# Ghoul-tn/DSTAGNN_Drought

Measured on AMD Instinct MI355X. Metric: DSTAGNN_block fwd+bwd samples/sec (B,N=170,T=12) @1/2/4/8 GPU; %HBM roofline, higher is better.
Workload: dtype fp32; 1 GPU; PEMS08 inner DSTAGNN_block fwd+bwd (train mode, dropout 0.05); global_batch=32, per_gpu_batch=32, N=170, T=12, F=32, K=3, n_heads=3, d_model=512, d_k=32, parallelism=dp1

## Files before the change

dstagnn_drought_amd/csrc/block.hip:

```cpp
#include <algorithm>
#include <atomic>
#include <vector>
#include <cstring>
#include <mutex>
#include <string>

#include "common.hpp"
#include <chrono>
#include <cstdio>
#include <initializer_list>
#include <map>
#include <utility>
#include "ops.hpp"
#include "streams.hpp"

static thread_local std::string g_last_error;
void set_last_error(const std::string& s) { g_last_error = s; }

namespace {

struct Arena {
  char* base;
  size_t off = 0;
  explicit Arena(void* b) : base((char*)b) {}
  float* take(size_t floats) {
    off = (off + 255) & ~size_t(255);
    float* p = base ? (float*)(base + off) : nullptr;
    off += floats * sizeof(float);
    return p;
  }
};

constexpr size_t kGemmWs = size_t(8) << 20;
constexpr size_t kPart = size_t(2) << 20;

struct Dims {
  int B, N, F, T, h, dk, dv, D, K, C;
  int64_t FT, BFT, BN, NN, HQ, HV, QW, KD, KC, CT, KCT, S;
  int Tg[3], ks[3];
  bool first, sparse, flash;
  bool fsmall;
  bool agg;
  bool dth;
  bool tfused;
  int NP;
  bool tfused_bwd;
  bool gfused;
  bool gbfused;
  int64_t tf_wg;
  int64_t nnz;
  int64_t apa_nnz;
};

Dims mkdims(const dstagnn_block_dims& d) {
  Dims m;
  m.B = d.B; m.N = d.N; m.F = d.F; m.T = d.T; m.h = d.n_heads; m.dk = d.d_k; m.dv = d.d_v;
  m.D = d.d_model; m.K = d.K; m.C = d.C;
  m.FT = (int64_t)m.F * m.T; m.BFT = (int64_t)m.B * m.FT; m.BN = (int64_t)m.B * m.N; m.NN = (int64_t)m.N * m.N;
  m.HQ = (int64_t)m.h * m.dk; m.HV = (int64_t)m.h * m.dv; m.QW = 2 * m.HQ + m.HV; m.KD = (int64_t)m.K * m.dk;
  m.KC = (int64_t)m.K * m.C; m.CT = (int64_t)m.C * m.T; m.KCT = m.KC * m.T; m.S = 3 * (int64_t)m.T - 12;
  for (int g = 0; g < 3; ++g) { m.ks[g] = 3 + 2 * g; m.Tg[g] = m.T - m.ks[g] + 1; }
  m.first = (m.F == 1);
  m.sparse = d.cheb_sparse != 0;
  m.flash = m.sparse && d.cheb_flash != 0;
  m.nnz = m.flash ? d.cheb_nnz : 0;
  m.fsmall = m.flash && flash_small(m.N);
  static const bool agg_env = env_flag("DSTAGNN_CHEB_AGG", true);
  m.agg = agg_env && m.sparse && cheb_agg_ok(m.F, m.C, m.K, m.T);
  m.dth = m.agg && cheb_agg_dtheta_fused(m.B, m.N, m.F, m.C, m.K, m.T, (int64_t)kGemmWs);
  m.apa_nnz = m.fsmall ? std::max(d.cheb_apa_nnz, 0) : 0;
  m.tfused = tat_fused_fwd_ok(m.N, m.T, m.h, m.dk, m.dv);
  m.NP = m.tfused ? tat_fused_np(m.N) : 0;
  m.tfused_bwd = m.tfused && tat_fused_bwd_ok(m.N, m.T, m.h, m.dk, m.dv, m.F, d.res_mode);
  m.tf_wg = m.tfused_bwd ? tat_fused_bwd_wgs(m.BFT) : 0;
  m.gfused = gtu_fused_fwd_ok(m.C, m.T);
  m.gbfused = gtu_fused_bwd_ok(m.C, m.T);
  return m;
}

struct SaveBufs {
  float *Wqkv, *Wqk, *Wp, *thcat, *Wgf[3], *Wgb[3];
  float* Wqkv_p;
  float *WfcT, *WqT;
  float* Wgt[3];
  float *E, *qkv, *att, *ctx, *u_tat, *mu_tat, *rs_tat, *O, *u_s, *mu_s, *rs_s, *Zd, *qk, *P, *W, *xth, *X;
  float *lse, *psupp, *wsupp;
  float *am, *amt, *papa;
  float* conv[3];
  float *G, *tco, *r, *mu_c, *rs_c, *u_et, *mu_et, *rs_et;
};

SaveBufs plan_save(const Dims& m, Arena& a) {
  SaveBufs s;
  s.Wqkv = a.take(m.QW * m.N);
  s.Wqkv_p = m.tfused ? a.take(m.QW * m.NP) : nullptr;
  s.WfcT = m.tfused_bwd ? a.take(m.HV * m.NP) : nullptr;
  s.WqT = m.tfused_bwd ? a.take(m.QW * m.NP) : nullptr;
  for (int g = 0; g < 3; ++g) s.Wgt[g] = m.gfused ? a.take(2 * (int64_t)m.C * m.C * m.ks[g]) : nullptr;
  s.Wqk = a.take(2 * m.KD * m.D);
  s.Wp = a.take((int64_t)m.D * m.FT);
  s.thcat = a.take((int64_t)m.F * m.KC);
  for (int g = 0; g < 3; ++g) s.Wgf[g] = a.take(2 * (int64_t)m.C * m.C * m.ks[g]);
// ... 29 lines not shown
  s.rs_c = a.take(m.BN * m.T);
  if (m.first) {
    s.u_et = a.take((int64_t)m.B * m.T * m.N);
    s.mu_et = a.take((int64_t)m.B * m.T);
    s.rs_et = a.take((int64_t)m.B * m.T);
  } else {
    s.u_et = s.mu_et = s.rs_et = nullptr;
  }
  return s;
}

struct Scratch {
  float *gemm_ws, *part;
  float *gemm_ws_side, *part_side, *dWqkv, *dWqk;
  float *dtc, *dX, *gpre, *gcon_t, *bcon_t, *dres_t, *gcon_s, *bcon_s, *gcon_a, *gcon_e, *dconv[3], *dW, *dxth,
      *dthcat, *dqk, *dZd, *dY, *dWp, *dO, *dU, *dE, *dctx, *dqkv, *dscore, *du_et, *dGt;
  float *dzs, *dzs_r, *cc;
};

Scratch plan_scratch(const Dims& m, Arena& a) {
  Scratch s;
  s.gemm_ws = a.take(kGemmWs);
  s.part = a.take(kPart);
  s.dtc = a.take(m.BN * m.CT);
  s.dX = a.take(m.BN * m.CT);
  s.gpre = a.take(m.BN * m.CT);
  s.gemm_ws_side = a.take(kGemmWs);
  s.part_side = a.take(kPart);
  s.dWqkv = a.take(m.QW * m.N);
  s.dWqk = a.take(2 * m.KD * m.D);
  s.gcon_t = a.take(m.gbfused ? std::max<int64_t>(m.BN * m.CT, gtu_fused_bwd_part_floats(m.BN)) : m.BN * m.CT);
  s.bcon_t = a.take(m.BN * m.CT);
  s.dres_t = a.take(m.BN * m.CT);
  s.gcon_s = a.take(m.BN * m.D);
  s.bcon_s = a.take(m.BN * m.D);
  s.gcon_a = a.take(m.BFT * m.N);
  s.gcon_e = m.first ? a.take((int64_t)m.B * m.T * m.N) : nullptr;
  for (int g = 0; g < 3; ++g) s.dconv[g] = a.take((m.BN * m.T + m.ks[g] - 1) * 2 * m.C);
  s.dW = m.flash ? nullptr : a.take((int64_t)m.B * m.K * m.NN);
  s.dzs = m.flash ? a.take((int64_t)m.B * m.K * m.nnz) : nullptr;
  s.dzs_r = m.fsmall ? a.take((int64_t)m.B * m.K * m.nnz) : nullptr;
  s.cc = m.flash ? a.take((int64_t)m.B * m.K * m.N) : nullptr;
  s.dxth = m.agg ? nullptr : a.take(m.BN * m.KCT);
  s.dthcat = a.take((int64_t)m.F * m.KC);
  s.dqk = a.take(m.BN * 2 * m.KD);
  s.dZd = a.take(m.BN * m.D);
  s.dY = a.take(m.BN * m.D);
  s.dWp = a.take((int64_t)m.D * m.FT);
  s.dO = a.take(m.BFT * m.N);
  s.dU = a.take(m.BFT * m.N);
  s.dE = a.take(m.BFT * m.N);
  s.dctx = a.take(m.BFT * m.HV);
  s.dqkv = a.take(m.BFT * m.QW);
  s.dscore = a.take(m.BFT * m.h * m.T);
  s.du_et = m.first ? a.take((int64_t)m.B * m.T * m.N) : nullptr;
  s.dGt = gtu_tail_bwd_split(m.C, m.T) ? a.take(m.BN * m.C * m.S) : nullptr;
  return s;
}

struct WorkBufs {
  SaveBufs s;
  Scratch w;
};

WorkBufs plan_work(const Dims& m, Arena& a) {
  WorkBufs k{};
  SaveBufs& s = k.s;
  s.Wqkv = m.tfused ? nullptr : a.take(m.QW * m.N);
// ... 407 lines not shown
    }
    add(0, p.sat_wq, s.Wqk, m.KD * m.D, 0, 0, 0, 0);
    add(0, p.sat_wk, s.Wqk, m.KD * m.D, 0, 0, 0, m.KD * m.D);
    add(1, p.pre_conv_w, s.Wp, (int64_t)m.D * m.FT, m.F, m.T);
    for (int k = 0; k < m.K; ++k) add(2, p.theta[k], s.thcat, (int64_t)m.F * m.C, m.C, (int)m.KC, k);
    for (int g = 0; g < 3; ++g) {
      const int64_t n = 2 * (int64_t)m.C * m.C * m.ks[g];
      if (m.gfused) add(3, p.gtu_w[g], s.Wgt[g], n, m.C, m.ks[g]);
      if (!m.gfused || (m.gbfused && !lean)) add(7, p.gtu_w[g], s.Wgf[g], n, m.C, m.ks[g]);
      if (!m.gbfused && !lean) add(4, p.gtu_w[g], s.Wgb[g], n, m.C, m.ks[g]);
    }
    if (m.fsmall)
      for (int k = 0; k < m.K; ++k) {
        add(5, p.mask[k], s.am + (int64_t)k * m.NN, m.NN).src2 = gr.adj_pa;
        if (!lean) add(6, p.mask[k], s.amt + (int64_t)k * m.NN, m.NN, m.N).src2 = gr.adj_pa;
      }
    if (full) {
      set_last_error("param_prep: more parameter re-layouts than kPrepSegsHost");
      return DSTAGNN_E_ARG;
    }
    DS_TRY(op_param_prep(pp, st));
    return 0;
  }

  int stage_sat() {
    {
      LnFwd a;
      a.R = (int)m.BN; a.L = m.D;
      a.src[0].p = s.u_s; a.src[0].row = idx1(m.D);
      a.src[1].p = p.embS_pos; a.src[1].row = idx2(m.N, m.D, 0);
      a.nsrc = 2;
      a.g = p.embS_g; a.b = p.embS_b;
      a.y = s.Zd; a.yrow = idx1(m.D);
      a.u = lean ? nullptr : s.u_s; a.mu = s.mu_s; a.rs = s.rs_s;
      if (d.train && d.drop_p > 0.f) {
        a.drop_p = d.drop_p; a.seed = d.seed; a.which = 0; a.drop_off = drop_off(d, 0);
      }
      DS_TRY(op_ln_fwd(a, st));
    }
    {
      Gemm g;
      g.M = (int)m.BN; g.N = (int)(2 * m.KD); g.K = m.D;
      g.A = s.Zd; g.am = idx1(m.D); g.ak = idx1(1);
      g.B = s.Wqk; g.bk = idx1(1); g.bn = idx1(m.D);
      g.C = s.qk; g.cm = idx1(2 * m.KD); g.cn = idx1(1);
      DS_TRY(run_gemm(g, w.gemm_ws, kGemmWs, st));
    }
    if (!m.flash) {
      Gemm g;
      g.M = m.N; g.N = m.N; g.K = m.dk; g.batch = m.B * m.K;
      g.A = s.qk; g.am = idx1(2 * m.KD); g.ak = idx1(1); g.az = idx2(m.K, m.dk, m.N * 2 * m.KD);
      g.B = s.qk; g.b_off = m.KD; g.bk = idx1(1); g.bn = idx1(2 * m.KD); g.bz = idx2(m.K, m.dk, m.N * 2 * m.KD);
      g.C = s.P; g.cm = idx1(m.N); g.cn = idx1(1); g.cz = idx1(m.NN);
      g.alpha = 1.f / sqrtf((float)m.dk);
      DS_TRY(run_gemm(g, w.gemm_ws, kGemmWs, st));
    }
    return 0;
  }

  ChebIO cheb_io() {
    ChebIO c;
    c.B = m.B; c.N = m.N; c.F = m.F; c.T = m.T; c.K = m.K; c.C = m.C;
    c.x = x; c.S = s.P; c.mask = p.mask; c.g = &gr; c.sparse = m.sparse; c.thcat = s.thcat;
    c.P = s.P; c.W = s.W; c.xth = m.dth ? nullptr : s.xth; c.X = s.X;
    c.agg = m.agg;
    if (m.flash) {
      fl = make_fl(m, p, gr, s);
// ... 102 lines not shown
  const float* dout;
  const float* dre;
  float* dx;
  float* dres;
  SaveBufs& s;
  Scratch& w;
  hipStream_t st;
  Streams ks;
  ChebFl fl;
  ChebFl flash_args() {
    ChebFl f = make_fl(m, p, gr, s);
    f.dzs = w.dzs; f.dzs_r = w.dzs_r; f.cc = w.cc; f.dqk = w.dqk;
    for (int k = 0; k < m.K; ++k) f.dmask[k] = gd.mask[k];
    return f;
  }
  int fork() { return ks.fork(); }
  int join() { return ks.join(); }
  SyncTok dx_ready;
  int mark_side(SyncTok* t) {
    *t = SyncTok{};
    if (!ks.split()) return 0;
    return ks.signal(ks.sd, t);
  }
  int wait_side(const SyncTok& t) {
    if (!ks.split()) return 0;
    return ks.wait(st, t);
  }

  float* preconv_bias_part() const {
    const int64_t pb = ln_bwd_part_blocks(m.BN);
    if (!gd.pre_conv_b || !ln_bwd_partials_ok(m.D) || 2 * pb > m.BN) return nullptr;
    return w.gcon_s + pb * m.D;
  }
  bool tat_part() const { return ln_bwd_partials_ok(m.N) && 2 * ln_bwd_part_blocks(m.BFT) <= m.BFT; }

  int colsum_on(hipStream_t q, const float* in, int64_t A, int O, int I, float* out) {
    if (!out) return 0;
    float* part = q == st ? w.part : w.part_side;
    return op_colsum(in, A, O, I, out, 1, 0.f, part, kPart, q);
  }
  int colsums(std::initializer_list<std::pair<const float*, float*>> io, int64_t A, int O, int I,
              bool on_main = false) {
    const hipStream_t q = on_main ? st : ks.side();
    const float* ins[4];
    float* outs[4];
    int n = 0;
    for (const auto& q : io)
      if (q.second && n < 4) { ins[n] = q.first; outs[n] = q.second; ++n; }
    if (!n) return 0;
    return op_colsum_multi(ins, outs, n, A, O, I, 1, 0.f, q == st ? w.part : w.part_side, kPart, q);
  }
  int gemm(const Gemm& g, ForkSig* sig = nullptr) { return run_gemm(g, w.gemm_ws, kGemmWs, st, sig); }
  static constexpr int kSideSplitK = 192;
  int sgemm(const Gemm& g0) {
    Gemm g = g0;
    if (ks.split() && !g.splitk_target) g.splitk_target = kSideSplitK;
    return run_gemm(g, ks.split() ? w.gemm_ws_side : w.gemm_ws, kGemmWs, ks.side());
  }

  int stage_tail_fused() {
    GtuFusedBwdArgs g;
    g.BN = m.BN; g.C = m.C; g.T = m.T; g.first = m.first;
    g.dout = dout; g.r = s.r; g.tco = s.tco; g.mu = s.mu_c; g.rs = s.rs_c; g.x = x; g.X = s.X;
    for (int q = 0; q < 3; ++q) { g.conv[q] = s.conv[q]; g.wf[q] = s.Wgf[q]; g.dconv[q] = w.dconv[q]; }
    g.fcmy_w = p.fcmy_w; g.ln_g = p.ln_g; g.res_w = p.res_w;
    if (d.train && d.drop_p > 0.f) { g.drop_p = d.drop_p; g.seed = d.seed; g.drop_off = drop_off(d, 1); }
// ... 214 lines not shown
      g.A = w.dW; g.am = idx1(m.N); g.ak = idx1(1); g.az = idx1(m.NN);
      g.B = s.qk; g.b_off = m.KD; g.bk = idx1(ld); g.bn = idx1(1); g.bz = idx2(m.K, m.dk, m.N * ld);
      g.C = w.dqk; g.cm = idx1(ld); g.cn = idx1(1); g.cz = idx2(m.K, m.dk, m.N * ld);
      g.alpha = sc;
      DS_TRY(gemm(g));
    }
    if (!m.flash) {
      Gemm g;
      g.M = m.N; g.N = m.dk; g.K = m.N; g.batch = m.B * m.K;
      g.A = w.dW; g.am = idx1(1); g.ak = idx1(m.N); g.az = idx1(m.NN);
      g.B = s.qk; g.bk = idx1(ld); g.bn = idx1(1); g.bz = idx2(m.K, m.dk, m.N * ld);
      g.C = w.dqk; g.c_off = m.KD; g.cm = idx1(ld); g.cn = idx1(1); g.cz = idx2(m.K, m.dk, m.N * ld);
      g.alpha = sc;
      DS_TRY(gemm(g));
    }
    const int64_t ln_rows = ln_bwd_partials_ok(m.D) ? ln_bwd_part_blocks(m.BN) : m.BN;
    {
      Gemm g;
      g.M = (int)m.BN; g.N = m.D; g.K = (int)ld;
      g.A = w.dqk; g.am = idx1(ld); g.ak = idx1(1);
      g.B = s.Wqk; g.bk = idx1(m.D); g.bn = idx1(1);
      g.C = w.dZd; g.cm = idx1(m.D); g.cn = idx1(1);
      DS_TRY(gemm(g));
    }
    {
      LnBwd a;
      a.R = (int)m.BN; a.L = m.D;
      a.dy = w.dZd; a.dyrow = idx1(m.D);
      a.u = s.u_s; a.mu = s.mu_s; a.rs = s.rs_s; a.g = p.embS_g;
      if (d.train && d.drop_p > 0.f) {
        a.drop_p = d.drop_p; a.seed = d.seed; a.which = 0; a.drop_off = drop_off(d, 0);
      }
      a.dx = w.dY; a.dxrow = idx1(m.D);
      if (ln_bwd_partials_ok(m.D)) {
        a.gpart = w.gcon_s; a.bpart = w.bcon_s;
        a.xpart = preconv_bias_part();
      } else {
        a.gcontrib = w.gcon_s; a.bcontrib = w.bcon_s;
      }
      DS_TRY(op_ln_bwd(a, st));
    }
    DS_TRY(ks.fork_on([&](ForkSig* sig) -> int {
      DS_TRY(debug_delay(st, true));
      return stage_preconv(sig);
    }));
    if (gd.sat_wq || gd.sat_wk) {
      Gemm g;
      g.M = (int)ld; g.N = m.D; g.K = (int)m.BN;
      g.A = w.dqk; g.am = idx1(1); g.ak = idx1(ld);
      g.B = s.Zd; g.bk = idx1(m.D); g.bn = idx1(1);
      const bool adjacent = gd.sat_wq && gd.sat_wk == gd.sat_wq + m.KD * m.D;
      g.C = adjacent ? gd.sat_wq : w.dWqk; g.cm = idx1(m.D); g.cn = idx1(1);
      DS_TRY(sgemm(g));
      if (!adjacent) {
        PackRows pk;
        pk.n = 2; pk.cols = m.D; pk.unpack = 1;
        pk.src[0] = w.dWqk; pk.rows[0] = (int)m.KD; pk.rows[1] = (int)m.KD;
        pk.dst[0] = gd.sat_wq; pk.dst[1] = gd.sat_wk;
        DS_TRY(op_pack_rows(pk, ks.side()));
      }
    }
    float* xpart = preconv_bias_part();
    DS_TRY(colsums({{w.gcon_s, gd.embS_g}, {w.bcon_s, gd.embS_b}, {xpart, xpart ? gd.pre_conv_b : nullptr}},
                   ln_rows, m.D, 1));
    if (!xpart) DS_TRY(colsum_on(ks.side(), w.dY, m.BN, m.D, 1, gd.pre_conv_b));
    if (gd.embS_pos) DS_TRY(op_sum_middle(w.dY, 1, m.B, (int64_t)m.N * m.D, gd.embS_pos, 0.f, ks.side()));
    if (gd.pre_conv_w) DS_TRY(sgemm(dwp_gemm()));
    return 0;
  }

  Gemm dwp_gemm() {
    Gemm g;
    g.M = m.D; g.N = (int)m.FT; g.K = (int)m.BN;
    g.A = w.dY; g.am = idx1(1); g.ak = idx1(m.D);
    g.B = s.O; g.bk = idx1(1); g.bn = idx1(m.BN);
    g.C = gd.pre_conv_w; g.cm = idx1(m.FT); g.cn = idx2(m.T, m.F, 1);
    return g;
  }

  int stage_preconv(ForkSig* sig) {
    Gemm g;
    g.M = (int)m.FT; g.N = (int)m.BN; g.K = m.D;
    g.A = s.Wp; g.am = idx1(1); g.ak = idx1(m.FT);
    g.B = w.dY; g.bk = idx1(1); g.bn = idx1(m.D);
    g.C = w.dO; g.cm = idx1(m.BN); g.cn = idx1(1);
    return gemm(g, sig);
  }

  int stage_tat_fused() {
    const int64_t N = m.N;
    if (!m.first) DS_TRY(wait_side(dx_ready));
    TatFusedBwdArgs t;
    t.dO = w.dO; t.u = s.u_tat; t.mu = s.mu_tat; t.rs = s.rs_tat; t.g = p.tat_ln_g;
    t.gpart = w.gcon_a; t.bpart = w.gcon_a + tat_bslab() * N;
#ifdef DSTAGNN_RACEBUG_NOFORK
    t.ln_fold = 0;
#else
    t.ln_fold = 1;
#endif
// ... 212 lines not shown
int dstagnn_prof_records(dstagnn_prof_record* out, int cap) { return gemm_prof_records(out, cap < 0 ? 0 : cap); }
int dstagnn_version(void) { return 1; }

int dstagnn_block_sizes(const dstagnn_block_dims* d, size_t* save_bytes, size_t* scratch_bytes) {
  DS_TRY(check_dims(d));
  if (!save_bytes || !scratch_bytes) return DSTAGNN_E_ARG;
  plan_sizes(mkdims(*d), save_bytes, scratch_bytes);
  return 0;
}

int dstagnn_block_save_offset(const dstagnn_block_dims* d, int which, size_t* offset_bytes, size_t* count) {
  DS_TRY(check_dims(d));
  if (!offset_bytes || !count || which < 0 || which > 2) return DSTAGNN_E_ARG;
  const Dims m = mkdims(*d);
  Arena a((void*)(uintptr_t)256);
  SaveBufs s = plan_save(m, a);
  const float* t = which == 0 ? s.X : (which == 1 ? s.tco : s.r);
  *offset_bytes = (size_t)((const char*)t - (char*)(uintptr_t)256);
  *count = (size_t)(m.BN * m.CT);
  return 0;
}

int dstagnn_block_paths(const dstagnn_block_dims* d, uint32_t* bits) {
  DS_TRY(check_dims(d));
  if (!bits) return DSTAGNN_E_ARG;
  const Dims m = mkdims(*d);
  *bits = (m.sparse ? DSTAGNN_PATH_SPARSE : 0u) | (m.flash ? DSTAGNN_PATH_FLASH : 0u) |
          (m.fsmall ? DSTAGNN_PATH_FLASH_SMALL : 0u) | (m.agg ? DSTAGNN_PATH_CHEB_AGG : 0u) |
          (m.tfused ? DSTAGNN_PATH_TAT_FUSED_FWD : 0u) | (m.tfused_bwd ? DSTAGNN_PATH_TAT_FUSED_BWD : 0u) |
          (m.gfused ? DSTAGNN_PATH_GTU_FUSED_FWD : 0u) | (m.gbfused ? DSTAGNN_PATH_GTU_FUSED_BWD : 0u);
  return 0;
}

int dstagnn_block_forward(const dstagnn_block_dims* d, const dstagnn_block_params* p, const dstagnn_graph* g,
                          const float* x, const float* res_att, float* out, float* re_at, void* save,
                          size_t save_bytes, void* scratch, size_t scratch_bytes, dstagnn_stream_t stream) {
  DS_TRY(check_dims(d));
  if (!p || !g || !x || !out || !re_at || !save || !scratch) { set_last_error("null argument"); return DSTAGNN_E_ARG; }
  if (d->res_mode != DSTAGNN_RES_NONE && !res_att) { set_last_error("res_att missing"); return DSTAGNN_E_ARG; }
  Dims m = mkdims(*d);
  DS_TRY(check_space(m, save_bytes, scratch_bytes));
  DS_TRY(check_graph(m, g));
  Arena a(align256(save)), b(align256(scratch));
  SaveBufs s = plan_save(m, a);
  Scratch w = plan_scratch(m, b);
  Fwd f{m, *d, *p, *g, x, d->res_mode ? res_att : nullptr, out, re_at, s, w, (hipStream_t)stream};
  return f.run();
}

int dstagnn_block_forward_only_size(const dstagnn_block_dims* d, size_t* work_bytes) {
  DS_TRY(check_dims(d));
  if (!work_bytes) return DSTAGNN_E_ARG;
  *work_bytes = plan_work_size(mkdims(*d));
  return 0;
}

int dstagnn_block_forward_only(const dstagnn_block_dims* d, const dstagnn_block_params* p, const dstagnn_graph* g,
                               const float* x, const float* res_att, float* out, float* re_at, void* work,
                               size_t work_bytes, dstagnn_stream_t stream) {
  DS_TRY(check_dims(d));
  if (!p || !g || !x || !out || !re_at || !work) { set_last_error("null argument"); return DSTAGNN_E_ARG; }
  if (d->res_mode != DSTAGNN_RES_NONE && !res_att) { set_last_error("res_att missing"); return DSTAGNN_E_ARG; }
  Dims m = mkdims(*d);
  if (work_bytes < plan_work_size(m)) {
    set_last_error("work smaller than dstagnn_block_forward_only_size()");
    return DSTAGNN_E_SPACE;
// ... 150 lines not shown
```

dstagnn_drought_amd/csrc/ops.hip:

```cpp
#include <map>
#include <mutex>

#include "common.hpp"
#include "handoff.hpp"
#include "ops.hpp"

namespace {

__global__ __launch_bounds__(256) void transpose_kernel(const float* __restrict__ in, float* __restrict__ out,
                                                        int R, int Cc, int64_t in_bs, int64_t out_bs, float beta) {
  __shared__ float tile[32][33];
  const int b = blockIdx.z;
  const int r0 = blockIdx.y * 32, c0 = blockIdx.x * 32;
  const float* ip = in + (int64_t)b * in_bs;
  float* op = out + (int64_t)b * out_bs;
  const int tx = threadIdx.x & 31, ty = threadIdx.x >> 5;
  float old[4] = {0.f, 0.f, 0.f, 0.f};
  if (beta != 0.f) {
#pragma unroll
    for (int u = 0; u < 4; ++u) {
      const int c = c0 + ty + 8 * u, r = r0 + tx;
      if (r < R && c < Cc) old[u] = op[(int64_t)c * R + r];
    }
  }
// ... 211 lines not shown
      red[0][wv][lane + 64 * q] = gp[q];
      red[1][wv][lane + 64 * q] = bp[q];
    }
    __syncthreads();
    for (int e4 = threadIdx.x; e4 < L / 4; e4 += 256) {
      float4 g = red[0][0][e4], b = red[1][0][e4];
#pragma unroll
      for (int k = 1; k < 4; ++k) {
        const float4 g2 = red[0][k][e4], b2 = red[1][k][e4];
        g.x += g2.x; g.y += g2.y; g.z += g2.z; g.w += g2.w;
        b.x += b2.x; b.y += b2.y; b.z += b2.z; b.w += b2.w;
      }
      if (a.gpart) reinterpret_cast<float4*>(a.gpart + (int64_t)blockIdx.x * L)[e4] = g;
      if (a.bpart) reinterpret_cast<float4*>(a.bpart + (int64_t)blockIdx.x * L)[e4] = b;
    }
    if (a.xpart) {
      __syncthreads();
#pragma unroll
      for (int q = 0; q < V4; ++q) red[0][wv][lane + 64 * q] = xp[q];
      __syncthreads();
      for (int e4 = threadIdx.x; e4 < L / 4; e4 += 256) {
        float4 x = red[0][0][e4];
#pragma unroll
        for (int k = 1; k < 4; ++k) {
          const float4 x2 = red[0][k][e4];
          x.x += x2.x; x.y += x2.y; x.z += x2.z; x.w += x2.w;
        }
        reinterpret_cast<float4*>(a.xpart + (int64_t)blockIdx.x * L)[e4] = x;
      }
    }
  }
}

static bool al16p(const void* p) { return (reinterpret_cast<uintptr_t>(p) & 15) == 0; }
static bool map4(const Idx2& m) { return m.s0 % 4 == 0 && m.s1 % 4 == 0; }
static bool ln_v4_env() {
  static const bool on = env_flag("DSTAGNN_LN_V4", true);
  return on;
}
static bool ln_fwd_v4_ok(const LnFwd& a) {
  if (!ln_v4_env() || (a.L != 256 && a.L != 512 && a.L != 1024) || a.yes != 1 || !map4(a.yrow)) return false;
  for (int s = 0; s < a.nsrc; ++s)
    if (a.src[s].es != 1 || !map4(a.src[s].row) || !al16p(a.src[s].p)) return false;
  return al16p(a.g) && al16p(a.b) && al16p(a.y) && al16p(a.u);
}
static bool ln_bwd_v4_ok(const LnBwd& a) {
  return ln_v4_env() && (a.L == 256 || a.L == 512 || a.L == 1024) && a.dyes == 1 && a.dxes == 1 && map4(a.dyrow) &&
         map4(a.dxrow) && al16p(a.dy) && al16p(a.u) && al16p(a.g) && al16p(a.dx) && al16p(a.gpart) &&
         al16p(a.bpart) && al16p(a.xpart);
}

__device__ __forceinline__ float wg_sum4(float v, float* red4) {
  v = wave_sum(v);
  const int w = threadIdx.x >> 6;
  if ((threadIdx.x & 63) == 0) red4[w] = v;
  __syncthreads();
  const float t = (red4[0] + red4[1]) + (red4[2] + red4[3]);
  __syncthreads();
  return t;
}

template <int VPT, int NSRC>
__global__ __launch_bounds__(256) void ln_fwd_wg_kernel(LnFwd a) {
  __shared__ float red4[4];
  const int tid = threadIdx.x, row = blockIdx.x, L = a.L;
  float xs[NSRC][VPT], gv[VPT], bv[VPT], v[VPT];
#pragma unroll
  for (int q = 0; q < VPT; ++q) {
    const int e = min(tid + 256 * q, L - 1);
#pragma unroll
    for (int s = 0; s < NSRC; ++s) xs[s][q] = a.src[s].p[ioff(a.src[s].row, row) + (int64_t)e * a.src[s].es];
    gv[q] = a.g[e];
    bv[q] = a.b[e];
  }
  float sum = 0.f;
#pragma unroll
  for (int q = 0; q < VPT; ++q) {
    float u = 0.f;
#pragma unroll
    for (int s = 0; s < NSRC; ++s) u += xs[s][q];
    v[q] = tid + 256 * q < L ? u : 0.f;
    sum += v[q];
  }
// ... 664 lines not shown
  dim3 grid((unsigned)cdiv64(a.R, 4));
  if (ln_fwd_v4_ok(a)) {
#define DS_LN4(V) \
    if (a.nsrc == 1) hipLaunchKernelGGL((ln_fwd_v4_kernel<V, 1>), grid, dim3(256), 0, st, a); \
    else if (a.nsrc == 2) hipLaunchKernelGGL((ln_fwd_v4_kernel<V, 2>), grid, dim3(256), 0, st, a); \
    else hipLaunchKernelGGL((ln_fwd_v4_kernel<V, 3>), grid, dim3(256), 0, st, a);
    if (a.L == 256) { DS_LN4(1) } else if (a.L == 512) { DS_LN4(2) } else { DS_LN4(4) }
#undef DS_LN4
    DS_CHECK_LAUNCH();
    return 0;
  }
  int vpt = (int)cdiv64(a.L, 64);
  if (vpt <= 1) launch_ln_fwd<1>(a, grid, st);
  else if (vpt <= 2) launch_ln_fwd<2>(a, grid, st);
  else if (vpt <= 4) launch_ln_fwd<4>(a, grid, st);
  else if (vpt <= 8) launch_ln_fwd<8>(a, grid, st);
  else if (vpt <= 16) launch_ln_fwd<16>(a, grid, st);
  else if (a.L <= 4096) {
    const dim3 g((unsigned)a.R);
    const int v = (int)cdiv64(a.L, 256);
#define DS_LNW(V) \
  if (a.nsrc == 1) hipLaunchKernelGGL((ln_fwd_wg_kernel<V, 1>), g, dim3(256), 0, st, a); \
  else if (a.nsrc == 2) hipLaunchKernelGGL((ln_fwd_wg_kernel<V, 2>), g, dim3(256), 0, st, a); \
  else hipLaunchKernelGGL((ln_fwd_wg_kernel<V, 3>), g, dim3(256), 0, st, a);
    if (v <= 8) { DS_LNW(8) } else { DS_LNW(16) }
#undef DS_LNW
  }
  else { set_last_error("ln_fwd: row too long"); return DSTAGNN_E_SHAPE; }
  DS_CHECK_LAUNCH();
  return 0;
}

int op_ln_bwd(const LnBwd& a, hipStream_t st) {
  int vpt = (int)cdiv64(a.L, 64);
  if (a.gpart || a.bpart || a.xpart) {
    if (!ln_bwd_partials_ok(a.L)) { set_last_error("ln_bwd: partial slabs need L <= 1024"); return DSTAGNN_E_SHAPE; }
    dim3 grid((unsigned)ln_bwd_part_blocks(a.R));
    if (kLnRowsPerWave == 1 && ln_bwd_v4_ok(a)) {
      if (a.L == 256) hipLaunchKernelGGL((ln_bwd_v4_kernel<1, true>), grid, dim3(256), 0, st, a);
      else if (a.L == 512) hipLaunchKernelGGL((ln_bwd_v4_kernel<2, true>), grid, dim3(256), 0, st, a);
      else hipLaunchKernelGGL((ln_bwd_v4_kernel<4, true>), grid, dim3(256), 0, st, a);
      DS_CHECK_LAUNCH();
      return 0;
    }
    if (vpt <= 1) hipLaunchKernelGGL((ln_bwd_kernel<1, true>), grid, dim3(256), 0, st, a);
    else if (vpt <= 2) hipLaunchKernelGGL((ln_bwd_kernel<2, true>), grid, dim3(256), 0, st, a);
    else if (vpt <= 4) hipLaunchKernelGGL((ln_bwd_kernel<4, true>), grid, dim3(256), 0, st, a);
    else if (vpt <= 8) hipLaunchKernelGGL((ln_bwd_kernel<8, true>), grid, dim3(256), 0, st, a);
    else hipLaunchKernelGGL((ln_bwd_kernel<16, true>), grid, dim3(256), 0, st, a);
    DS_CHECK_LAUNCH();
    return 0;
  }
  dim3 grid((unsigned)cdiv64(a.R, 4));
  if (vpt <= 1) hipLaunchKernelGGL((ln_bwd_kernel<1, false>), grid, dim3(256), 0, st, a);
  else if (vpt <= 2) hipLaunchKernelGGL((ln_bwd_kernel<2, false>), grid, dim3(256), 0, st, a);
  else if (vpt <= 4) hipLaunchKernelGGL((ln_bwd_kernel<4, false>), grid, dim3(256), 0, st, a);
  else if (vpt <= 8) hipLaunchKernelGGL((ln_bwd_kernel<8, false>), grid, dim3(256), 0, st, a);
  else if (vpt <= 16) hipLaunchKernelGGL((ln_bwd_kernel<16, false>), grid, dim3(256), 0, st, a);
  else if (a.L <= 4096) {
    if (a.L <= 2048) hipLaunchKernelGGL((ln_bwd_wg_kernel<8>), dim3((unsigned)a.R), dim3(256), 0, st, a);
    else hipLaunchKernelGGL((ln_bwd_wg_kernel<16>), dim3((unsigned)a.R), dim3(256), 0, st, a);
  }
  else { set_last_error("ln_bwd: row too long"); return DSTAGNN_E_SHAPE; }
  DS_CHECK_LAUNCH();
  return 0;
}
// ... 132 lines not shown
```

dstagnn_drought_amd/csrc/ops.hpp:

```cpp
#pragma once
#include "common.hpp"

struct LnSrc {
  const float* p = nullptr;
  Idx2 row;
  int64_t es = 1;
};

struct LnFwd {
  int R = 0, L = 0;
  LnSrc src[3];
  int nsrc = 0;
  const float* g = nullptr;
  const float* b = nullptr;
  float eps = 1e-5f;
  float* y = nullptr; Idx2 yrow; int64_t yes = 1;
  float* u = nullptr;
  float* mu = nullptr; float* rs = nullptr;
  float drop_p = 0.f; uint64_t seed = 0; uint32_t which = 0;
  uint64_t drop_off = 0;
};

struct LnBwd {
  int R = 0, L = 0;
  const float* dy = nullptr; Idx2 dyrow; int64_t dyes = 1;
  const float* u = nullptr; const float* mu = nullptr; const float* rs = nullptr; const float* g = nullptr;
  float drop_p = 0.f; uint64_t seed = 0; uint32_t which = 0;
  uint64_t drop_off = 0;
  float* dx = nullptr; Idx2 dxrow; int64_t dxes = 1; float beta = 0.f;
  float* gcontrib = nullptr;
  float* bcontrib = nullptr;
  float* gpart = nullptr;
  float* bpart = nullptr;
  float* xpart = nullptr;
};
constexpr int kLnRowsPerWave = 1;
inline int64_t ln_bwd_part_blocks(int64_t R) { return (R + 4 * kLnRowsPerWave - 1) / (4 * kLnRowsPerWave); }
inline bool ln_bwd_partials_ok(int L) { return L <= 1024; }

struct ChebSm {
  int B = 0, K = 0, N = 0;
  const float* S = nullptr;
  const float* apa = nullptr;
  const float* mask[DSTAGNN_MAX_K] = {};
  const float* cheb = nullptr;
  float* P = nullptr;
  float* W = nullptr;
  const float* dW = nullptr;
  float* dz = nullptr;
  float* dmask[DSTAGNN_MAX_K] = {};
};

struct ColsumArgs {
  const float* in[4] = {};
  float* out[4] = {};
  int nsrc = 1;
  int64_t A = 0; int O = 0, I = 1;
  int64_t achunk = 1;
  int64_t ostride = 1; float beta = 0.f;
  float* part = nullptr; int P = 1; int OL = 1;
};

struct PackRows {
  int n = 0, cols = 0, unpack = 0;
  int rows[8] = {};
  const float* src[8] = {};
  float* dst[8] = {};
};
// ... 256 lines not shown
```

dstagnn_drought_amd/csrc/torch_ops.cpp:

```cpp
#include <ATen/ATen.h>
#include <c10/core/DeviceGuard.h>
#include <c10/hip/HIPStream.h>
#include <torch/autograd.h>
#include <torch/library.h>

#include <cmath>
#include <cstring>
#include <vector>

#include "../../include/dstagnn.h"

using at::Tensor;
using torch::autograd::AutogradContext;
using torch::autograd::variable_list;

namespace {

dstagnn_stream_t stream_of(const Tensor& t) {
  return (dstagnn_stream_t)c10::hip::getCurrentHIPStream(t.device().index()).stream();
}

void check_rc(int rc, const char* what) {
  TORCH_CHECK(rc == 0, what, " failed (code ", rc, "): ", dstagnn_last_error());
}
// ... 1010 lines not shown
           "dstagnn_emd_dense");
  return {out, st};
}

Tensor fast_stag_distances(const Tensor& coords, const Tensor& feats, double max_distance) {
  check_dev(coords, at::kDouble, "coords");
  check_dev(feats, at::kDouble, "feats");
  const int64_t N = coords.size(0);
  TORCH_CHECK(feats.size(0) == N, "coords and features disagree on the node count");
  c10::DeviceGuard guard(coords.device());
  Tensor sta = at::empty({N, N}, coords.options());
  check_rc(dstagnn_fast_stag_distances(coords.data_ptr<double>(), (int)N, (int)coords.size(1),
                                       feats.data_ptr<double>(), (int)feats.size(1), max_distance,
                                       sta.data_ptr<double>(), stream_of(coords)),
           "dstagnn_fast_stag_distances");
  return sta;
}

std::tuple<Tensor, Tensor, Tensor> graph_topk(const Tensor& sta, int64_t k, int64_t mode) {
  check_dev(sta, at::kDouble, "sta");
  const int64_t N = sta.size(0);
  c10::DeviceGuard guard(sta.device());
  Tensor A = at::empty({N, N}, sta.options()), R = at::empty({N, N}, sta.options());
  Tensor nbr = at::empty({N, k}, sta.options().dtype(at::kInt));
  check_rc(dstagnn_graph_topk(sta.data_ptr<double>(), (int)N, (int)k, (int)mode, A.data_ptr<double>(),
                              R.data_ptr<double>(), nbr.data_ptr<int32_t>(), stream_of(sta)),
           "dstagnn_graph_topk");
  return {A, R, nbr};
}

int64_t library_version() { return dstagnn_version(); }

int64_t set_splitk_target(int64_t target) { return dstagnn_set_splitk_target((int)target); }
int64_t set_gemm_bf16(int64_t on) { return dstagnn_set_gemm_bf16((int)on); }

void prof_start(int64_t capacity) { check_rc(dstagnn_prof_start((int)capacity), "dstagnn_prof_start"); }
std::vector<double> prof_stop() {
  dstagnn_prof_stats s{};
  check_rc(dstagnn_prof_stop(&s), "dstagnn_prof_stop");
  return {s.launches, s.flops, s.bytes, s.ms, s.max_ms, s.dropped};
}
std::vector<double> prof_records() {
  const int n = dstagnn_prof_records(nullptr, 0);
  std::vector<dstagnn_prof_record> r((size_t)std::max(n, 0));
  if (n > 0) dstagnn_prof_records(r.data(), n);
  std::vector<double> out;
  out.reserve(4 * r.size());
  for (const auto& x : r) {
    out.push_back((double)x.kind);
    out.push_back(x.flops);
    out.push_back(x.bytes);
    out.push_back(x.ms);
  }
  return out;
}

}

TORCH_LIBRARY(dstagnn, m) {
  m.class_<BlockPlan>("BlockPlan")
      .def(torch::init<std::vector<Tensor>, std::vector<int64_t>, std::vector<Tensor>, std::vector<int64_t>>());
  m.def("block_planned(Tensor x, Tensor? res_att, __torch__.torch.classes.dstagnn.BlockPlan plan, Tensor anchor, "
        "float drop_p, int seed, int flags) -> (Tensor, Tensor)");
#define DSTAGNN_BLK_ARGS \
  "Tensor x, Tensor? res_att, Tensor[] params, int[] slots, Tensor[] graph, int[] cfg, float drop_p, int seed, int flags"
  m.def("block(" DSTAGNN_BLK_ARGS ") -> (Tensor, Tensor)");
// ... 17 lines not shown
  m.def("colsum(Tensor x, int O, int I) -> Tensor");
  m.def("head_fwd(Tensor[] outs, Tensor w1, Tensor b1, Tensor w2, Tensor b2) -> (Tensor, Tensor)");
  m.def("head_bwd(Tensor[] outs, Tensor w1, Tensor w2, Tensor h, Tensor dy, int[] need) -> Tensor[]");
  m.def("adam_step(Tensor(a!)[] params, Tensor[] grads, Tensor(b!)[] exp_avgs, Tensor(c!)[] exp_avg_sqs, "
        "float beta1, float beta2, float eps, float step_size, float bc2_sqrt) -> ()");
  m.def("grad_sumsq(Tensor[] grads) -> Tensor");
  m.def("adam_step_ex(Tensor(a!)[] params, Tensor[] grads, Tensor(b!)[] exp_avgs, Tensor(c!)[] exp_avg_sqs, "
        "float beta1, float beta2, float eps, float step_size, float bc2_sqrt, float lr, float weight_decay, "
        "bool decoupled, float max_norm, bool skip_nonfinite, Tensor stat, Tensor(d!) skipped) -> ()");
  m.def("grad_scale(Tensor(a!)[] grads, Tensor stat, float max_norm) -> ()");
  m.def("loss_fwd(Tensor y, Tensor target, int kind, float param, int mask_mode, float null_val) -> (Tensor, Tensor)");
  m.def("loss_bwd(Tensor y, Tensor target, Tensor stat, Tensor? gout, int kind, float param, int mask_mode, "
        "float null_val) -> Tensor");
  m.def("metrics_update(Tensor pred, Tensor target, float null_val, Tensor(a!) table) -> ()");
  m.def("window_gather(Tensor series, Tensor rel, Tensor labels, Tensor idx, Tensor mean, Tensor std, int P) "
        "-> (Tensor, Tensor)");
  m.def("window_stats(Tensor series, Tensor w, float wtotal) -> Tensor");
  m.def("window_tile_nodes(int F, int Tin) -> int", window_tile_nodes);
  m.def("window_stats_masked(Tensor series, Tensor w, float null_val) -> (Tensor, Tensor)");
  m.def("window_fill_forward(Tensor series, float null_val, int max_gap) -> (Tensor, Tensor)");
  m.def("window_fill_chunk() -> int", window_fill_chunk);
  m.def("window_fill_cols() -> int", window_fill_cols);
  m.def("window_gather_masked(Tensor xsrc, Tensor ysrc, Tensor rel, Tensor labels, Tensor idx, Tensor mean, "
        "Tensor std, int P, float null_val) -> (Tensor, Tensor)");
  m.def("stag_prep(Tensor data) -> (Tensor, Tensor, Tensor)");
  m.def("stag_emd_pairs(Tensor xhat, Tensor p, Tensor psum, Tensor pairs, bool with_pivots) -> (Tensor, Tensor, Tensor)");
  m.def("stag_emd_lds_bytes(int T, int F) -> int", stag_emd_lds_bytes);
  m.def("emd_dense(Tensor p, Tensor q, Tensor D) -> (Tensor, Tensor)");
  m.def("fast_stag_distances(Tensor coords, Tensor feats, float max_distance) -> Tensor");
  m.def("graph_topk(Tensor sta, int k, int mode) -> (Tensor, Tensor, Tensor)");
  m.def("version() -> int", library_version);
  m.def("prof_start(int capacity) -> ()", prof_start);
  m.def("set_splitk_target(int target) -> int", set_splitk_target);
  m.def("set_gemm_bf16(int on) -> int", set_gemm_bf16);
  m.def("prof_stop() -> float[]", prof_stop);
  m.def("prof_records() -> float[]", prof_records);
}

TORCH_LIBRARY_IMPL(dstagnn, CUDA, m) {
  m.impl("block", block_infer);
  m.impl("block_planned", block_planned_infer);
  m.impl("block_fwd", block_fwd);
  m.impl("block_fwd_only", block_fwd_only);
  m.impl("block_fwd_only_bytes", block_fwd_only_bytes);
  m.impl("block_bwd", block_bwd);
  m.impl("block_time_stage", block_time_stage);
  m.impl("dropout_masks", dropout_masks);
  m.impl("block_cheb_out", block_cheb_out);
  m.impl("block_relu_out", block_relu_out);
  m.impl("block_paths", block_paths);
  m.impl("cheb_sat_fwd", cheb_sat_fwd);
  m.impl("cheb_sat_bwd", cheb_sat_bwd);
  m.impl("gemm_f32", gemm_f32);
  m.impl("colsum", colsum);
  m.impl("head_fwd", head_fwd);
  m.impl("head_bwd", head_bwd);
  m.impl("adam_step", adam_step);
  m.impl("grad_sumsq", grad_sumsq);
  m.impl("adam_step_ex", adam_step_ex);
  m.impl("grad_scale", grad_scale);
  m.impl("loss_fwd", loss_fwd);
  m.impl("loss_bwd", loss_bwd);
  m.impl("metrics_update", metrics_update);
  m.impl("window_gather", window_gather);
  m.impl("window_stats", window_stats);
  m.impl("window_stats_masked", window_stats_masked);
// ... 14 lines not shown
```

include/dstagnn.h:

```cpp
#ifndef DSTAGNN_H
#define DSTAGNN_H

#include <stddef.h>
#include <stdint.h>

#ifdef __cplusplus
extern "C" {
#endif

typedef void* dstagnn_stream_t;

#define DSTAGNN_MAX_K 8
#define DSTAGNN_HEAD_MAX_BLOCKS 16

enum {
  DSTAGNN_OK = 0,
  DSTAGNN_E_SHAPE = 10001,
  DSTAGNN_E_ARG = 10002,
  DSTAGNN_E_SPACE = 10003
};

enum { DSTAGNN_RES_NONE = 0, DSTAGNN_RES_BCAST = 1, DSTAGNN_RES_FULL = 2 };

typedef struct dstagnn_block_dims {
// ... 72 lines not shown
  const float* tsupp;
  const int* csc2csr;
  const int* apa_idx;
  const int* apa2t;
} dstagnn_graph;

int dstagnn_block_sizes(const dstagnn_block_dims* d, size_t* save_bytes, size_t* scratch_bytes);

int dstagnn_block_forward(const dstagnn_block_dims* d, const dstagnn_block_params* p, const dstagnn_graph* g,
                          const float* x, const float* res_att, float* out, float* re_at,
                          void* save, size_t save_bytes, void* scratch, size_t scratch_bytes,
                          dstagnn_stream_t stream);

int dstagnn_block_forward_only_size(const dstagnn_block_dims* d, size_t* work_bytes);
int dstagnn_block_forward_only(const dstagnn_block_dims* d, const dstagnn_block_params* p, const dstagnn_graph* g,
                               const float* x, const float* res_att, float* out, float* re_at,
                               void* work, size_t work_bytes, dstagnn_stream_t stream);

int dstagnn_block_save_offset(const dstagnn_block_dims* d, int which, size_t* offset_bytes, size_t* count);

enum {
  DSTAGNN_PATH_SPARSE = 1,
  DSTAGNN_PATH_FLASH = 2,
  DSTAGNN_PATH_FLASH_SMALL = 4,
  DSTAGNN_PATH_CHEB_AGG = 8,
  DSTAGNN_PATH_TAT_FUSED_FWD = 16,
  DSTAGNN_PATH_TAT_FUSED_BWD = 32,
  DSTAGNN_PATH_GTU_FUSED_FWD = 64,
  DSTAGNN_PATH_GTU_FUSED_BWD = 128,
  DSTAGNN_PATH_SAT_LN_FUSED = 256
};
int dstagnn_block_paths(const dstagnn_block_dims* d, uint32_t* bits);

int dstagnn_block_backward(const dstagnn_block_dims* d, const dstagnn_block_params* p, const dstagnn_graph* g,
                           const float* x, const float* res_att, const float* d_out, const float* d_re_at,
                           float* d_x, float* d_res_att, const dstagnn_block_grads* grads,
                           void* save, size_t save_bytes, void* scratch, size_t scratch_bytes,
                           dstagnn_stream_t stream);


int dstagnn_cheb_sat_forward(int B, int N, int F, int T, int K, int C, int sparse,
                             const float* x, const float* sat, const float* theta_cat, const float* mask_cat,
                             const dstagnn_graph* g, float* out,
                             float* P, float* W, float* xth, void* scratch, size_t scratch_bytes,
                             dstagnn_stream_t stream);
int dstagnn_cheb_sat_backward(int B, int N, int F, int T, int K, int C, int sparse,
                              const float* x, const float* theta_cat, const dstagnn_graph* g,
                              const float* out, const float* P, const float* W, const float* xth,
                              const float* d_out, float* d_x, float* d_sat, float* d_theta_cat, float* d_mask_cat,
                              void* scratch, size_t scratch_bytes, dstagnn_stream_t stream);

typedef struct dstagnn_idx { int64_t div, s0, s1; } dstagnn_idx;
typedef struct dstagnn_gemm_desc {
  int M, N, K, batch;
  const float* A; dstagnn_idx a_m, a_k, a_z; int64_t a_off;
  const float* B; dstagnn_idx b_k, b_n, b_z; int64_t b_off;
  float* C;       dstagnn_idx c_m, c_n, c_z; int64_t c_off;
  float alpha, beta;
  const float* bias; int64_t bias_stride;
  int relu;
} dstagnn_gemm_desc;
int dstagnn_gemm_f32(const dstagnn_gemm_desc* g, void* scratch, size_t scratch_bytes, dstagnn_stream_t stream);

int dstagnn_colsum(const float* in, int64_t A, int O, int I, float* out, int64_t ostride, float beta,
                   void* scratch, size_t scratch_bytes, dstagnn_stream_t stream);

// ... 143 lines not shown
```

Measured before the change: 61770 samples/s.

## Add node-periodic LayerNorm backward kernel fusing pos-embedding and bias reductions

```diff
diff --git a/dstagnn_drought_amd/csrc/block.hip b/dstagnn_drought_amd/csrc/block.hip
--- a/dstagnn_drought_amd/csrc/block.hip
+++ b/dstagnn_drought_amd/csrc/block.hip
@@ -42,6 +42,8 @@
   bool fsmall;
   bool agg;
   bool dth;
+  bool lnn;
+  int64_t lns;
   bool tfused;
   int NP;
   bool tfused_bwd;
@@ -68,6 +70,8 @@
   static const bool agg_env = env_flag("DSTAGNN_CHEB_AGG", true);
   m.agg = agg_env && m.sparse && cheb_agg_ok(m.F, m.C, m.K, m.T);
   m.dth = m.agg && cheb_agg_dtheta_fused(m.B, m.N, m.F, m.C, m.K, m.T, (int64_t)kGemmWs);
+  m.lnn = ln_bwd_nodes_shape_ok(m.BN, m.D, m.N);
+  m.lns = m.lnn ? ln_bwd_nodes_slices(m.BN, m.N) : 0;
   m.apa_nnz = m.fsmall ? std::max(d.cheb_apa_nnz, 0) : 0;
   m.tfused = tat_fused_fwd_ok(m.N, m.T, m.h, m.dk, m.dv);
   m.NP = m.tfused ? tat_fused_np(m.N) : 0;
@@ -163,8 +167,8 @@
   s.gcon_t = a.take(m.gbfused ? std::max<int64_t>(m.BN * m.CT, gtu_fused_bwd_part_floats(m.BN)) : m.BN * m.CT);
   s.bcon_t = a.take(m.BN * m.CT);
   s.dres_t = a.take(m.BN * m.CT);
-  s.gcon_s = a.take(m.BN * m.D);
-  s.bcon_s = a.take(m.BN * m.D);
+  s.gcon_s = a.take(m.lnn ? 2 * m.lns * m.N * m.D : m.BN * m.D);
+  s.bcon_s = a.take(m.lnn ? m.lns * m.N * m.D : m.BN * m.D);
   s.gcon_a = a.take(m.BFT * m.N);
   s.gcon_e = m.first ? a.take((int64_t)m.B * m.T * m.N) : nullptr;
   for (int g = 0; g < 3; ++g) s.dconv[g] = a.take((m.BN * m.T + m.ks[g] - 1) * 2 * m.C);
@@ -638,7 +642,7 @@
       a.nsrc = 2;
       a.g = p.embS_g; a.b = p.embS_b;
       a.y = s.Zd; a.yrow = idx1(m.D);
-      a.u = lean ? nullptr : s.u_s; a.mu = s.mu_s; a.rs = s.rs_s;
+      a.u = lean || m.lnn ? nullptr : s.u_s; a.mu = s.mu_s; a.rs = s.rs_s;
       if (d.train && d.drop_p > 0.f) {
         a.drop_p = d.drop_p; a.seed = d.seed; a.which = 0; a.drop_off = drop_off(d, 0);
       }
@@ -807,6 +811,10 @@
     if (!gd.pre_conv_b || !ln_bwd_partials_ok(m.D) || 2 * pb > m.BN) return nullptr;
     return w.gcon_s + pb * m.D;
   }
+  float* embs_possum() const {
+    if (!gd.embS_pos && !gd.pre_conv_b) return nullptr;
+    return m.lns == 1 && gd.embS_pos ? gd.embS_pos : w.gcon_s + m.lns * m.N * m.D;
+  }
   bool tat_part() const { return ln_bwd_partials_ok(m.N) && 2 * ln_bwd_part_blocks(m.BFT) <= m.BFT; }
 
   int colsum_on(hipStream_t q, const float* in, int64_t A, int O, int I, float* out) {
@@ -1087,7 +1095,11 @@
         a.drop_p = d.drop_p; a.seed = d.seed; a.which = 0; a.drop_off = drop_off(d, 0);
       }
       a.dx = w.dY; a.dxrow = idx1(m.D);
-      if (ln_bwd_partials_ok(m.D)) {
+      if (m.lnn) {
+        a.period = m.N; a.pos = p.embS_pos;
+        a.gpart = w.gcon_s; a.bpart = w.bcon_s;
+        a.possum = embs_possum();
+      } else if (ln_bwd_partials_ok(m.D)) {
         a.gpart = w.gcon_s; a.bpart = w.bcon_s;
         a.xpart = preconv_bias_part();
       } else {
@@ -1115,11 +1127,19 @@
         DS_TRY(op_pack_rows(pk, ks.side()));
       }
     }
-    float* xpart = preconv_bias_part();
-    DS_TRY(colsums({{w.gcon_s, gd.embS_g}, {w.bcon_s, gd.embS_b}, {xpart, xpart ? gd.pre_conv_b : nullptr}},
-                   ln_rows, m.D, 1));
-    if (!xpart) DS_TRY(colsum_on(ks.side(), w.dY, m.BN, m.D, 1, gd.pre_conv_b));
-    if (gd.embS_pos) DS_TRY(op_sum_middle(w.dY, 1, m.B, (int64_t)m.N * m.D, gd.embS_pos, 0.f, ks.side()));
+    if (m.lnn) {
+      float* possum = embs_possum();
+      DS_TRY(colsums({{w.gcon_s, gd.embS_g}, {w.bcon_s, gd.embS_b}, {possum, possum ? gd.pre_conv_b : nullptr}},
+                     m.lns * m.N, m.D, 1));
+      if (m.lns > 1 && gd.embS_pos)
+        DS_TRY(op_sum_middle(possum, 1, (int)m.lns, (int64_t)m.N * m.D, gd.embS_pos, 0.f, ks.side()));
+    } else {
+      float* xpart = preconv_bias_part();
+      DS_TRY(colsums({{w.gcon_s, gd.embS_g}, {w.bcon_s, gd.embS_b}, {xpart, xpart ? gd.pre_conv_b : nullptr}},
+                     ln_rows, m.D, 1));
+      if (!xpart) DS_TRY(colsum_on(ks.side(), w.dY, m.BN, m.D, 1, gd.pre_conv_b));
+      if (gd.embS_pos) DS_TRY(op_sum_middle(w.dY, 1, m.B, (int64_t)m.N * m.D, gd.embS_pos, 0.f, ks.side()));
+    }
     if (gd.pre_conv_w) DS_TRY(sgemm(dwp_gemm()));
     return 0;
   }
@@ -1398,6 +1418,14 @@
   return 0;
 }
 
+int dstagnn_ln_bwd_nodes_ok(int64_t rows, int L, int64_t period, int64_t dy_row_stride, int64_t dx_row_stride,
+                            int64_t ptr_misalign) {
+  return ln_bwd_nodes_shape_ok(rows, L, period) && dy_row_stride == L && dx_row_stride == L &&
+                 (ptr_misalign & 15) == 0
+             ? 1
+             : 0;
+}
+
 int dstagnn_block_forward(const dstagnn_block_dims* d, const dstagnn_block_params* p, const dstagnn_graph* g,
                           const float* x, const float* res_att, float* out, float* re_at, void* save,
                           size_t save_bytes, void* scratch, size_t scratch_bytes, dstagnn_stream_t stream) {
diff --git a/dstagnn_drought_amd/csrc/ops.hip b/dstagnn_drought_amd/csrc/ops.hip
--- a/dstagnn_drought_amd/csrc/ops.hip
+++ b/dstagnn_drought_amd/csrc/ops.hip
@@ -267,6 +267,113 @@
   }
 }
 
+__device__ __forceinline__ float4 ld4_any(const float* p) { return make_float4(p[0], p[1], p[2], p[3]); }
+__device__ __forceinline__ void f4acc(float4& s, const float4& v) { s.x += v.x; s.y += v.y; s.z += v.z; s.w += v.w; }
+
+
+template <int V4, int W>
+__global__ __launch_bounds__(64 * W) void ln_bwd_nodes_kernel(LnBwd a) {
+  const int lane = threadIdx.x & 63, wv = threadIdx.x >> 6;
+  constexpr int L = 256 * V4;
+  const int j = blockIdx.x, sl = blockIdx.y;
+  const int64_t P = a.period;
+  const int nb = min((int)(a.R / P), (sl + 1) * 2 * W);
+  const bool haspos = a.pos != nullptr;
+  float4 gp[V4], bp[V4], xp[V4], gl[V4], pl[V4];
+  const DropKey dk = drop_key(a.seed, a.which);
+  const bool drop = a.drop_p > 0.f;
+  const float dthr = drop ? a.drop_p : -1.0f, dscale = drop ? 1.0f / (1.0f - a.drop_p) : 1.0f;
+  struct Row {
+    float4 dy[V4], u[V4];
+    float mean, rs;
+  };
+  auto load = [&](Row& r, int b) {
+    const int64_t row = (int64_t)b * P + j, ro = row * L;
+#pragma unroll
+    for (int q = 0; q < V4; ++q) {
+      const int e4 = lane + 64 * q;
+      r.dy[q] = reinterpret_cast<const float4*>(a.dy + ro)[e4];
+      r.u[q] = reinterpret_cast<const float4*>(a.u + ro)[e4];
+    }
+    r.mean = a.mu[row];
+    r.rs = a.rs[row];
+  };
+  auto process = [&](const Row& r, int b) {
+#pragma clang fp contract(off)
+    const int64_t row = (int64_t)b * P + j;
+    const float mean = r.mean, rs = r.rs;
+    float4 dyv[V4], xh[V4];
+    float s1 = 0.f, s2 = 0.f;
+#pragma unroll
+    for (int q = 0; q < V4; ++q) {
+      const int e4 = lane + 64 * q;
+#pragma unroll
+      for (int c = 0; c < 4; ++c) {
+        float dy = f4at(r.dy[q], c);
+        dy *= drop_u(dk, (uint64_t)row * L + 4 * e4 + c + a.drop_off) >= dthr ? dscale : 0.0f;
+        float u = f4at(r.u[q], c);
+        if (haspos) u += f4at(pl[q], c);
+        const float x = (u - mean) * rs;
+        l4set(dyv[q], c, dy);
+        l4set(xh[q], c, x);
+        const float dxh = dy * f4at(gl[q], c);
+        s1 = __builtin_fmaf(dy, f4at(gl[q], c), s1);
+        s2 = __builtin_fmaf(dxh, x, s2);
+      }
+    }
+    s1 = wave_sum(s1) / L;
+    s2 = wave_sum(s2) / L;
+#pragma unroll
+    for (int q = 0; q < V4; ++q) {
+      float4 d, gx;
+#pragma unroll
+      for (int c = 0; c < 4; ++c) {
+        const float t = rs * __builtin_fmaf(-s2, f4at(xh[q], c), __builtin_fmaf(f4at(dyv[q], c), f4at(gl[q], c), -s1));
+        l4set(d, c, t);
+        l4set(gx, c, f4at(dyv[q], c) * f4at(xh[q], c));
+      }
+      reinterpret_cast<float4*>(a.dx + row * L)[lane + 64 * q] = d;
+      f4acc(gp[q], gx);
+      f4acc(bp[q], dyv[q]);
+      f4acc(xp[q], d);
+    }
+  };
+  const int b = sl * 2 * W + wv;
+  const bool one = b < nb, two = b + W < nb;
+  Row r0, r1;
+  load(r0, one ? b : sl * 2 * W);
+  load(r1, two ? b + W : sl * 2 * W);
+  const float* prow = haspos ? a.pos + (int64_t)j * L : a.g;
+#pragma unroll
+  for (int q = 0; q < V4; ++q) {
+    const int e4 = lane + 64 * q;
+    gp[q] = bp[q] = xp[q] = make_float4(0.f, 0.f, 0.f, 0.f);
+    gl[q] = ld4_any(a.g + 4 * e4);
+    pl[q] = ld4_any(prow + 4 * e4);
+  }
+  __builtin_amdgcn_sched_barrier(0);
+  if (one) process(r0, b);
+  if (two) process(r1, b + W);
+  __shared__ float4 red[3][W][64 * V4];
+#pragma unroll
+  for (int q = 0; q < V4; ++q) {
+    red[0][wv][lane + 64 * q] = gp[q];
+    red[1][wv][lane + 64 * q] = bp[q];
+    red[2][wv][lane + 64 * q] = xp[q];
+  }
+  __syncthreads();
+  for (int i = threadIdx.x; i < 3 * (L / 4); i += 64 * W) {
+    const int what = i / (L / 4), e4 = i % (L / 4);
+    float* out = what == 0 ? a.gpart : what == 1 ? a.bpart : a.possum;
+    if (!out) continue;
+    float4 s = red[what][0][e4];
+#pragma unroll
+    for (int k = 1; k < W; ++k) f4acc(s, red[what][k][e4]);
+    float* o = out + ((int64_t)sl * P + j) * L + 4 * e4;
+    o[0] = s.x; o[1] = s.y; o[2] = s.z; o[3] = s.w;
+  }
+}
+
 static bool al16p(const void* p) { return (reinterpret_cast<uintptr_t>(p) & 15) == 0; }
 static bool map4(const Idx2& m) { return m.s0 % 4 == 0 && m.s1 % 4 == 0; }
 static bool ln_v4_env() {
@@ -284,6 +391,21 @@
          map4(a.dxrow) && al16p(a.dy) && al16p(a.u) && al16p(a.g) && al16p(a.dx) && al16p(a.gpart) &&
          al16p(a.bpart) && al16p(a.xpart);
 }
+static bool rows_of(const Idx2& m, int L) { return !m.two && m.s0 == L; }
+
+}
+
+bool ln_bwd_nodes_shape_ok(int64_t R, int L, int64_t period) {
+  return ln_v4_env() && (L == 256 || L == 512 || L == 1024) && period > 0 && R > 0 && R % period == 0 &&
+         R <= 0x7fffffff && period <= 0x7fffffff && ln_bwd_nodes_slices(R, period) <= 65535;
+}
+bool ln_bwd_nodes_ok(const LnBwd& a) {
+  return ln_bwd_nodes_shape_ok(a.R, a.L, a.period) && a.dyes == 1 && a.dxes == 1 && rows_of(a.dyrow, a.L) &&
+         rows_of(a.dxrow, a.L) && a.beta == 0.f && !a.gcontrib && !a.bcontrib && !a.xpart && al16p(a.dy) &&
+         al16p(a.u) && al16p(a.dx) && al16p(a.gpart) && al16p(a.bpart);
+}
+
+namespace {
 
 __device__ __forceinline__ float wg_sum4(float v, float* red4) {
   v = wave_sum(v);
@@ -1014,6 +1136,16 @@
 }
 
 int op_ln_bwd(const LnBwd& a, hipStream_t st) {
+  if (a.period > 0) {
+    if (!ln_bwd_nodes_ok(a)) { set_last_error("ln_bwd: shape refused by ln_bwd_nodes_ok"); return DSTAGNN_E_SHAPE; }
+    constexpr int W = kLnNodesWaves;
+    const dim3 grid((unsigned)a.period, (unsigned)ln_bwd_nodes_slices(a.R, a.period));
+    if (a.L == 256) hipLaunchKernelGGL((ln_bwd_nodes_kernel<1, W>), grid, dim3(64 * W), 0, st, a);
+    else if (a.L == 512) hipLaunchKernelGGL((ln_bwd_nodes_kernel<2, W>), grid, dim3(64 * W), 0, st, a);
+    else hipLaunchKernelGGL((ln_bwd_nodes_kernel<4, W>), grid, dim3(64 * W), 0, st, a);
+    DS_CHECK_LAUNCH();
+    return 0;
+  }
   int vpt = (int)cdiv64(a.L, 64);
   if (a.gpart || a.bpart || a.xpart) {
     if (!ln_bwd_partials_ok(a.L)) { set_last_error("ln_bwd: partial slabs need L <= 1024"); return DSTAGNN_E_SHAPE; }
diff --git a/dstagnn_drought_amd/csrc/ops.hpp b/dstagnn_drought_amd/csrc/ops.hpp
--- a/dstagnn_drought_amd/csrc/ops.hpp
+++ b/dstagnn_drought_amd/csrc/ops.hpp
@@ -33,7 +33,19 @@
   float* gpart = nullptr;
   float* bpart = nullptr;
   float* xpart = nullptr;
-};
+  int64_t period = 0;
+  const float* pos = nullptr;
+  float* possum = nullptr;
+};
+bool ln_bwd_nodes_ok(const LnBwd& a);
+bool ln_bwd_nodes_shape_ok(int64_t R, int L, int64_t period);
+#ifndef DSTAGNN_LN_NODES_WAVES
+#define DSTAGNN_LN_NODES_WAVES 4
+#endif
+constexpr int kLnNodesWaves = DSTAGNN_LN_NODES_WAVES;
+inline int64_t ln_bwd_nodes_slices(int64_t R, int64_t period) {
+  return (R / period + 2 * kLnNodesWaves - 1) / (2 * kLnNodesWaves);
+}
 constexpr int kLnRowsPerWave = 1;
 inline int64_t ln_bwd_part_blocks(int64_t R) { return (R + 4 * kLnRowsPerWave - 1) / (4 * kLnRowsPerWave); }
 inline bool ln_bwd_partials_ok(int L) { return L <= 1024; }
diff --git a/dstagnn_drought_amd/csrc/torch_ops.cpp b/dstagnn_drought_amd/csrc/torch_ops.cpp
--- a/dstagnn_drought_amd/csrc/torch_ops.cpp
+++ b/dstagnn_drought_amd/csrc/torch_ops.cpp
@@ -1066,6 +1066,9 @@
 int64_t library_version() { return dstagnn_version(); }
 
 int64_t set_splitk_target(int64_t target) { return dstagnn_set_splitk_target((int)target); }
+bool ln_bwd_nodes_ok(int64_t rows, int64_t L, int64_t period) {
+  return dstagnn_ln_bwd_nodes_ok(rows, (int)L, period, L, L, 0) != 0;
+}
 int64_t set_gemm_bf16(int64_t on) { return dstagnn_set_gemm_bf16((int)on); }
 
 void prof_start(int64_t capacity) { check_rc(dstagnn_prof_start((int)capacity), "dstagnn_prof_start"); }
@@ -1149,6 +1152,7 @@
   m.def("version() -> int", library_version);
   m.def("prof_start(int capacity) -> ()", prof_start);
   m.def("set_splitk_target(int target) -> int", set_splitk_target);
+  m.def("ln_bwd_nodes_ok(int rows, int L, int period) -> bool", ln_bwd_nodes_ok);
   m.def("set_gemm_bf16(int on) -> int", set_gemm_bf16);
   m.def("prof_stop() -> float[]", prof_stop);
   m.def("prof_records() -> float[]", prof_records);
diff --git a/include/dstagnn.h b/include/dstagnn.h
--- a/include/dstagnn.h
+++ b/include/dstagnn.h
@@ -128,6 +128,9 @@
 };
 int dstagnn_block_paths(const dstagnn_block_dims* d, uint32_t* bits);
 
+int dstagnn_ln_bwd_nodes_ok(int64_t rows, int L, int64_t period, int64_t dy_row_stride, int64_t dx_row_stride,
+                            int64_t ptr_misalign);
+
 int dstagnn_block_backward(const dstagnn_block_dims* d, const dstagnn_block_params* p, const dstagnn_graph* g,
                            const float* x, const float* res_att, const float* d_out, const float* d_re_at,
                            float* d_x, float* d_res_att, const dstagnn_block_grads* grads,
```

Result: no change. 62360 samples/s, median of 6 (+1.0%).
